# lightkurve/lightkurve

Hardware: NVIDIA H100
Metric: lombscargle_freqbins_x_cadences_per_s (higher is better)
Workload: dtype f32 spreading + FFT, f64 phase (nufft)

## Files before the change

lightkurve_b200/csrc/ls_nufft.cu:

```cuda
#include <algorithm>

#include "common.cuh"
#include "ls_common.cuh"
#include "nufft_core.h"
#include "nufft_v2.cuh"

namespace lkb {

using nufft::Cad;

namespace {

constexpr int GL_NQ = 48;
struct GlNodes {
  double x[GL_NQ], w[GL_NQ];
};

__global__ void nufft_cad_kernel(const double* __restrict__ t, int64_t N, double df, int64_t M, int w,
                                 Cad* __restrict__ cad, int* __restrict__ unsorted) {
  const int64_t n = (int64_t)blockIdx.x * blockDim.x + threadIdx.x;
  if (n >= N) return;
  cad[n] = nufft::cad_entry(t[n], df, M, w);
  if (n > 0 && t[n] < t[n - 1]) *unsorted = 1;
  if (t[n] < 0.0) *unsorted = 1;
// ... 722 lines not shown
  return LKB_OK;
}

int ls_nufft_run(const double* d_t, int64_t N, const float* d_yc, int64_t ystride, const float* d_ysumf,
                 const float* d_absmax, int B, const double* d_freq, int64_t F, const float4* d_rot,
                 const float2* d_rot2, int64_t F_low, int normalization, double norm_scale, float* d_pow,
                 cudaStream_t st, int ws_alt, bool prof) {
  const NufftPlan pl = g_plan;
  const int w = pl.w, p = pl.p;
  const float beta = pl.beta;
  const int64_t k0 = pl.k0, M = pl.M;
  const int npairs = (B + 1) / 2;
  const int mode = (pl.Wt != nullptr) ? 3 : fft_mode(p) == 3 ? 0 : fft_mode(p);
  const char* ve = getenv("LKB_NUFFT_VERIFY");
  const bool verify = ve && atoi(ve) != 0 && F_low < F;
  if (mode == 3) {
    const int64_t Mh = M >> 1;
    const size_t cells = (size_t)pl.n1max << V2_PB;
    float2 *T = nullptr, *G = nullptr;
    LKB_TRY(ws_get_t<float2>(ws_alt ? WS_OUT4 : WS_H, (size_t)B * Mh, &T));
    LKB_TRY(ws_get_t<float2>(ws_alt ? WS_OUT5 : WS_I, std::max((size_t)B * cells, verify ? (size_t)4 * Mh : (size_t)0), &G));
    unsigned* d_worst = nullptr;
    if (verify) LKB_TRY(ws_get_t<unsigned>(ws_alt ? WS_OUT7 : WS_OUT6, 1, &d_worst));
    const int ptc = V2_LOG_TILE - (p - 1 - V2_PB);
    if (prof) prof_begin(st);
    constexpr int LCS = 8;
    LKB_LAUNCH(dim3(blocks_for((int64_t)cells, 256), (unsigned)((B + LCS - 1) / LCS)), 256, st, nufft2_spread_kernel<LCS>)(
        pl.fge, pl.cad, pl.Wt, d_yc, ystride, B, w, p, ptc, pl.n1max, G);
    LKB_LAUNCH_CHECK();
    LKB_TRY(v2_cols(G, T, p, pl.n1max, B, pl.tb, st));
    const float esc_ratio = escalate_ratio();
    unsigned* d_peak = nullptr;
    int* d_list = nullptr;
    if (esc_ratio > 0.0f && F_low < F) {
      LKB_TRY(ws_get_t<unsigned>(ws_alt ? WS_Y3 : WS_Y2, (size_t)2 * B + 1, &d_peak));
      d_list = reinterpret_cast<int*>(d_peak + B);
      LKB_CUDA_CHECK(cudaMemsetAsync(d_peak, 0, sizeof(unsigned) * ((size_t)B + 1), st));
    }
    V2Finish fa;
    fa.ftab = pl.ftab; fa.k0 = k0; fa.F = F; fa.k_lo = F_low; fa.ysum = d_ysumf; fa.Nf = (float)N;
    fa.normalization = normalization; fa.scale = (float)norm_scale; fa.power = d_pow;
    fa.peak = d_peak; fa.lcmap = nullptr; fa.log2M = p;
    if (F_low < F) LKB_TRY(v2_rows(T, p, B, pl.tb, &fa, (float2*)nullptr, 0, st));
    if (F_low > 0) {
      double* acc = nullptr;
      LKB_TRY(ws_get_t<double>(ws_alt ? WS_X4 : WS_X3, (size_t)B * F_low * 2, &acc));
      LKB_CUDA_CHECK(cudaMemsetAsync(acc, 0, sizeof(double) * (size_t)B * F_low * 2, st));
// ... 3 lines not shown
          pl.lowD, N, pl.Npad, d_yc, ystride, B, (int)F_low, slice, acc);
      LKB_LAUNCH_CHECK();
      LKB_LAUNCH(blocks_for((int64_t)B * F_low, 256), 256, st, nufft2_lowfinish_kernel)(
          acc, B, (int)F_low, F, N, d_rot, d_rot2, d_ysumf, normalization, (float)norm_scale, d_pow, d_peak);
      LKB_LAUNCH_CHECK();
    }
    if (d_peak) {
      LKB_LAUNCH(blocks_for(B, 256), 256, st, nufft2_flag_kernel)(d_peak, d_absmax, B, (float)N, esc_ratio, d_list, d_list + 1,
                                                                pl.esc_total);
      LKB_LAUNCH_CHECK();
      int cap_max = 1024;
      if (const char* e = getenv("LKB_NUFFT_ESCALATE_CAP")) cap_max = std::max(1, atoi(e));
      const int cap = std::min(B, cap_max), gy = std::min(cap, 32);
      const size_t lowlen = F_low > 0 ? (size_t)F_low * 4 + (size_t)cap * F_low * 2 + cap : 0;
      double *Gbuf = nullptr;
      double2* Td = nullptr;
      LKB_TRY(ws_get_t<double>(ws_alt ? WS_Y6 : WS_Y4, 2 * (size_t)cap * cells + lowlen, &Gbuf));
      LKB_TRY(ws_get_t<double2>(ws_alt ? WS_Y7 : WS_Y5, (size_t)cap * Mh, &Td));
      double2* Gd = reinterpret_cast<double2*>(Gbuf);
      double* accW = Gbuf + 2 * (size_t)cap * cells;
      double* accY = accW + (size_t)F_low * 4;
      double* accS = accY + (size_t)cap * F_low * 2;
      const int* lst = d_list + 1;
      const int ptc_d = v2_log_tile(p - 1 - V2_PB, true) - (p - 1 - V2_PB);
      for (int base = 0; base < B; base += cap) {
        const V2Count nc = {d_list, base, cap};
        LKB_LAUNCH(dim3(blocks_for((int64_t)cells, 256), (unsigned)((gy + LCS_D - 1) / LCS_D)), 256, st,
                   nufft2_spread_list_kernel)(pl.fge, pl.cad, pl.Wtd, d_yc, ystride, lst, w, p, ptc_d, pl.n1max, Gd, nc);
        LKB_LAUNCH_CHECK();
        LKB_TRY(v2_cols(Gd, Td, p, pl.n1max, gy, pl.tbd, st, nc));
        V2Finish fd = fa;
        fd.peak = nullptr;
        fd.lcmap = lst;
        LKB_TRY(v2_rows(Td, p, gy, pl.tbd, &fd, (double2*)nullptr, 0, st, nc));
        if (F_low > 0) {
          LKB_CUDA_CHECK(cudaMemsetAsync(accW, 0, sizeof(double) * lowlen, st));
          LKB_LAUNCH(dim3((unsigned)F_low, blocks_for(N, 256 * LOWX_PER)), 256, st, nufft2_lowacc_kernel)(
              lst, nc, d_t, N, d_yc, ystride, d_freq, (int)F_low, accW, accY, accS);
          LKB_LAUNCH_CHECK();
          LKB_LAUNCH(blocks_for((int64_t)cap * F_low, 256), 256, st, nufft2_lowexact_finish_kernel)(
              lst, nc, accW, accY, accS, (int)F_low, F, N, normalization, (float)norm_scale, d_pow);
          LKB_LAUNCH_CHECK();
        }
      }
    }
    if (prof) prof_end(st);
    if (verify) {
      const int nv = std::min(B, 4);
      const int nk2 = (int)((k0 + F) >> (p - 1 - V2_PB)) + 1;
      LKB_TRY(v2_rows(T, p, nv, pl.tb, (const V2Finish*)nullptr, G, nk2, st));
      const char* fe = getenv("LKB_NUFFT_INJECT_FAULT");
// ... 145 lines not shown
  const int64_t pair = gid >> log2M, m = gid & (M - 1);
  const int64_t b0 = 2 * pair, b1 = b0 + 1;
  float2 v = make_float2(0.f, 0.f);
  {
    const int64_t po = poff[b0], n = off[b0 + 1] - off[b0];
    v.x = nufft::spread_cell_search(m, cad + po, n, y ? y + po : nullptr, y ? nufft::pow2_scale(absmax[b0]) : 1.0f, w,
                                    beta, M);
  }
  if (b1 < B) {
    const int64_t po = poff[b1], n = off[b1 + 1] - off[b1];
    v.y = nufft::spread_cell_search(m, cad + po, n, y ? y + po : nullptr, y ? nufft::pow2_scale(absmax[b1]) : 1.0f, w,
                                    beta, M);
  }
  Z[gid] = v;
}

__global__ void __launch_bounds__(256)
nufft2_spread_ragged_kernel(const Cad* __restrict__ cad, const float* __restrict__ y, const int64_t* __restrict__ off,
                            const int64_t* __restrict__ poff, int w, float beta, int p, int ptc, int n1max,
                            float2* __restrict__ G, const double* __restrict__ t, double df) {
  const int64_t cells = (int64_t)n1max << V2_PB;
  const int64_t e = (int64_t)blockIdx.x * blockDim.x + threadIdx.x;
  if (e >= cells) return;
  const int64_t M = (int64_t)1 << p, m = 2 * v2_zcell_of(e, ptc, n1max);
  const int64_t lc = blockIdx.y, po = poff[lc], n = off[lc + 1] - off[lc];
  float2 v;
  if (t) {
    const double dfM = df * (double)M;
    v.x = nufft::spread_cell_search_acc(m, cad + po, t + po, n, y ? y + po : nullptr, w, (double)beta, dfM, M);
    v.y = nufft::spread_cell_search_acc(m + 1, cad + po, t + po, n, y ? y + po : nullptr, w, (double)beta, dfM, M);
  } else {
    v.x = nufft::spread_cell_search(m, cad + po, n, y ? y + po : nullptr, 1.0f, w, beta, M);
    v.y = nufft::spread_cell_search(m + 1, cad + po, n, y ? y + po : nullptr, 1.0f, w, beta, M);
  }
  G[lc * cells + e] = v;
}

__device__ __forceinline__ float2 v2_unpack_real(const float2* __restrict__ Zn, int64_t kk, int64_t M) {
  const int64_t Mh = M >> 1;
  const float2 g1 = Zn[kk], g2 = Zn[(Mh - kk) & (Mh - 1)];
  const float2 E = make_float2(0.5f * (g1.x + g2.x), 0.5f * (g1.y - g2.y));
  const float2 O = make_float2(0.5f * (g1.y + g2.y), 0.5f * (g2.x - g1.x));
  double wsn, wcs;
  sincospi(2.0 * (double)kk / (double)M, &wsn, &wcs);
  const float wc = (float)wcs, ws = (float)wsn;
  return make_float2(E.x + wc * O.x - ws * O.y, E.y + wc * O.y + ws * O.x);
}

__device__ __forceinline__ float ragged_power(float2 hs, float2 win1, float2 win2, double Nd, double ysum,
                                              int normalization, double scale) {
  LsSums<double> d;
  d.zero();
  d.ch = (double)hs.x;
  d.sh = (double)hs.y;
  d.c = (double)win1.x;
  d.s = (double)win1.y;
  d.cc = 0.5 * (Nd + (double)win2.x);
  d.sc = 0.5 * (double)win2.y;
// ... 192 lines not shown
  const int64_t kmax = (int64_t)std::max(nterms, 1) * (k0 + F);
  const int64_t dec_first = nterms ? 0 : k0, dec_len = nterms ? kmax : F;
  LKB_TRY(ws_get_t<float2>(WS_IN4, dec_len, &dec));
  LKB_TRY(ws_get_t<float2>(WS_IN5, 2 * kmax, &dec2));
  LKB_TRY(ws_get_t<int>(WS_IN6, 1, &flag));

  LKB_CUDA_CHECK(cudaMemsetAsync(flag, 0, sizeof(int), st));
  {
    const unsigned gx = (unsigned)std::min<int64_t>(64, (nmax + 255) / 256);
    LKB_LAUNCH(dim3(gx ? gx : 1, (unsigned)B), 256, st, nufft_cad_ragged_kernel)(d_t, d_off, d_po, d_span, df, M, M2, w, cad,
                                                                          cad2, flag);
    LKB_LAUNCH_CHECK();
  }
  int h_flag = 0;
  LKB_CUDA_CHECK(cudaMemcpyAsync(&h_flag, flag, sizeof(int), cudaMemcpyDeviceToHost, st));
  LKB_CUDA_CHECK(cudaStreamSynchronize(st));
  if (h_flag) { set_error("NUFFT (ragged): a light curve has unsorted times"); return LKB_E_UNSUPPORTED; }
  LKB_LAUNCH(blocks_for(dec_len, 128), 128, st, nufft_deconv_kernel)(dec_first, dec_len, M, w, (double)beta, gl, dec);
  LKB_LAUNCH_CHECK();
  LKB_LAUNCH(blocks_for(2 * kmax, 128), 128, st, nufft_deconv_kernel)(0, 2 * kmax, M2, w, (double)beta, gl, dec2);
  LKB_LAUNCH_CHECK();

  const double* t_acc = getenv("LKB_NUFFT_RAGGED_W32") ? nullptr : d_t;
  const int ptc = V2_LOG_TILE - (p - 1 - V2_PB), ptc2 = V2_LOG_TILE - (p2 - 1 - V2_PB);
  const int nk2 = (int)(kmax >> (p - 1 - V2_PB)) + 1, nk2w = (int)((2 * kmax) >> (p2 - 1 - V2_PB)) + 1;
  prof_begin(st);
  for (int b0 = 0; b0 < B; b0 += group) {
    LKB_CHI2_OBSERVE(CHI2_PATH_GROUP);
    const int Bg = std::min(group, B - b0);
    const int64_t *off_g = d_off + b0, *po_g = d_po + b0;
    double span_min = 1e300;
    for (int b = b0; b < b0 + Bg; ++b) span_min = fmin(span_min, h_span[b]);
    const double nlow = floor((LS_LOWF_CYCLES / span_min - f0) / df) + 2.0;
    const int64_t F_low_max = nlow < 0.0 ? 0 : (nlow > (double)F ? F : (int64_t)nlow);
    LKB_LAUNCH(dim3(blocks_for((int64_t)cells2, 256), (unsigned)Bg), 256, st, nufft2_spread_ragged_kernel)(
        cad2, nullptr, off_g, po_g, w, beta, p2, ptc2, n1max2, G, t_acc, df);
    LKB_LAUNCH_CHECK();
    LKB_TRY(v2_cols(G, Tw, p2, n1max2, Bg, tb2, st));
    LKB_TRY(v2_rows(Tw, p2, Bg, tb2, nullptr, Zwn, nk2w, st));
    LKB_LAUNCH(dim3(blocks_for((int64_t)cells, 256), (unsigned)Bg), 256, st, nufft2_spread_ragged_kernel)(
        cad, d_y, off_g, po_g, w, beta, p, ptc, n1max, G, t_acc, df);
    LKB_LAUNCH_CHECK();
    LKB_TRY(v2_cols(G, T, p, n1max, Bg, tb, st));
    LKB_TRY(v2_rows(T, p, Bg, tb, nullptr, Zn, nk2, st));
    const double* ns_g = d_ns ? d_ns + b0 : nullptr;
    float* pow_g = d_pow + (size_t)b0 * F;
#define LKB_CHI2_FINISH(NT)                                                                                            \
// ... 202 lines not shown
```

lightkurve_b200/csrc/nufft_v2.cuh:

```cuda
#pragma once
#include "nufft_core.h"

namespace lkb {
namespace {

using nufft::V2_PB;
using nufft::V2_THREADS;
using nufft::V2_TILE;
constexpr int V2_LOG_TILE = 13;
static_assert((1 << V2_LOG_TILE) == V2_TILE, "tile size");
constexpr int V2_BC = 1 << V2_PB;
constexpr int V2_R = V2_TILE / (2 * V2_BC);
constexpr int V2_LSB = V2_BC + V2_BC / 16 + 1;
constexpr int V2R_P_MIN = V2_PB + 4 + 1, V2R_P_MAX = V2_PB + 13 + 1;

__host__ __device__ constexpr int v2_radix(int plog, int idx) {
  return (idx < plog / 4) ? 16 : ((idx == plog / 4 && (plog % 4)) ? (1 << (plog % 4)) : 0);
}
__host__ __device__ constexpr int v2_log2i(int r) { return r == 16 ? 4 : r == 8 ? 3 : r == 4 ? 2 : r == 2 ? 1 : 0; }
__host__ __device__ constexpr int v2_log_tile(int pa, bool dbl) { return (dbl && pa <= 12) ? 12 : V2_LOG_TILE; }
__device__ __forceinline__ int v2_skew(int a) { return a + (a >> 4); }
template <int nb>
__host__ __device__ constexpr int v2_in_off(int r) {
  return (nb % 16 == 0) ? r * (nb + nb / 16) : r * nb + ((r * nb) >> 4);
}

template <class CT>
__global__ void nufft2_tables_kernel(int pa, int pb, int ph, CT* __restrict__ tw_a, CT* __restrict__ tw_b,
                                     CT* __restrict__ t_hi, CT* __restrict__ t_lo) {
  const int la = nufft::v2_pass_table_len(pa), lb = nufft::v2_pass_table_len(pb), pl = nufft::v2_log2_lo(ph);
  const int nlo = 1 << pl, nhi = 1 << (ph - pl);
  int e = (int)(blockIdx.x * blockDim.x + threadIdx.x);
  int64_t num = 0, den = 1;
  CT* dst = nullptr;
  if (e < la) { nufft::v2_pass_table_entry(pa, e, &num, &den); dst = tw_a + e; }
  else if ((e -= la) < lb) { nufft::v2_pass_table_entry(pb, e, &num, &den); dst = tw_b + e; }
  else if ((e -= lb) < nhi) { num = e; den = nhi; dst = t_hi + e; }
  else if ((e -= nhi) < nlo) { num = e; den = (int64_t)1 << ph; dst = t_lo + e; }
  else return;
  double sn, cs;
  sincospi(2.0 * (double)num / (double)den, &sn, &cs);
  typedef typename nufft::CplxOf<CT>::real RT;
  *dst = nufft::CplxOf<CT>::mk((RT)cs, (RT)sn);
}

template <class RT>
__global__ void nufft2_weights_kernel(const double* __restrict__ t, int64_t N, double df, int64_t M, int w, double beta,
                                      RT* __restrict__ Wt) {
  const int64_t e = (int64_t)blockIdx.x * blockDim.x + threadIdx.x;
  if (e >= N * w) return;
  const int64_t n = e / w;
  const int q = (int)(e - n * w);
  const double x = df * t[n] * (double)M + (double)nufft::grid_shift(w);
  const double i0 = ceil(x - 0.5 * (double)w);
  const double z = (i0 + (double)q - x) * (2.0 / (double)w);
  const double s2 = 1.0 - z * z;
  Wt[e] = (s2 > 0.0) ? (RT)exp(beta * (sqrt(s2) - 1.0)) : (RT)0.0;
}

__device__ __forceinline__ int64_t v2_zcell_of(int64_t e, int ptc, int n1max) {
  const int64_t j = e & (((int64_t)1 << ptc) - 1), rest = e >> ptc;
  const int64_t n1 = rest % n1max, c = rest / n1max;
  return (n1 << V2_PB) + (c << ptc) + j;
}

template <int LCS>
__global__ void __launch_bounds__(256)
nufft2_spread_kernel(const int32_t* __restrict__ first_ge, const nufft::Cad* __restrict__ cad,
                     const float* __restrict__ Wt, const float* __restrict__ y, int64_t ystride, int B, int w, int p,
                     int ptc, int n1max, float2* __restrict__ G) {
  const int64_t cells = (int64_t)n1max << V2_PB;
  const int64_t e = (int64_t)blockIdx.x * blockDim.x + threadIdx.x;
  if (e >= cells) return;
  const int64_t M = (int64_t)1 << p, m = 2 * v2_zcell_of(e, ptc, n1max);
  const int lc0 = (int)blockIdx.y * LCS;
  const float* yr[LCS];
#pragma unroll
  for (int q = 0; q < LCS; ++q) {
    int b = lc0 + q;
    if (b > B - 1) b = B - 1;
    yr[q] = y + (int64_t)b * ystride;
  }
  float a0[LCS], a1[LCS];
#pragma unroll
  for (int q = 0; q < LCS; ++q) { a0[q] = 0.0f; a1[q] = 0.0f; }
  const int64_t L = nufft::table_len(M, w);
  for (int wrap = 0; wrap < 2; ++wrap) {
    const int64_t mm = m + (int64_t)wrap * M;
    if (mm + 1 >= L) break;
    int64_t lo_c = mm - w + 1, hi_c = mm + 2;
    if (lo_c < 0) lo_c = 0;
    if (hi_c > L - 1) hi_c = L - 1;
    const int32_t na = first_ge[lo_c], nb = first_ge[hi_c];
    for (int32_t n = na; n < nb; ++n) {
      const int tap = (int)(mm - (int64_t)cad[n].i0);
      const float* wr = Wt + (int64_t)n * w;
      const float w0 = (tap >= 0) ? wr[tap] : 0.0f;
      const float w1 = (tap + 1 < w) ? wr[tap + 1] : 0.0f;
#pragma unroll
      for (int q = 0; q < LCS; ++q) {
        const float v = yr[q][n];
        a0[q] = fmaf(w0, v, a0[q]);
        a1[q] = fmaf(w1, v, a1[q]);
      }
    }
  }
#pragma unroll
  for (int q = 0; q < LCS; ++q)
    if (lc0 + q < B) G[(int64_t)(lc0 + q) * cells + e] = make_float2(a0[q], a1[q]);
}

template <int PLOG, int LS, int IDX, int NS, class CT = float2, int NT = V2_THREADS>
__device__ __forceinline__ void v2_pass_t(CT* buf, const CT* __restrict__ tw, int nz = 1 << 30) {
  constexpr int R = v2_radix(PLOG, IDX);
  if constexpr (R != 0) {
    constexpr int LR = v2_log2i(R), NB = 16 / R, PNB = PLOG - LR, nb = 1 << PNB;
    constexpr bool WIDE = nb > NT;
    static_assert(WIDE || (NT % nb) == 0, "geometry");
    const int t = (int)threadIdx.x;
    CT u[NB][R];
    int base_in[NB];
#pragma unroll
    for (int q = 0; q < NB; ++q) {
      int line, i;
      if constexpr (WIDE) { line = 0; i = t + NT * q; }
      else { line = (t >> PNB) + ((NT * q) >> PNB); i = t & (nb - 1); }
      base_in[q] = line * LS + ((nb % 16 == 0) ? v2_skew(i) : i);
#pragma unroll
      for (int r = 0; r < R; ++r)
        u[q][r] = (IDX > 0 || r * nb < nz) ? buf[base_in[q] + v2_in_off<nb>(r)] : nufft::CplxOf<CT>::mk(0, 0);
    }
    __syncthreads();
#pragma unroll
    for (int q = 0; q < NB; ++q) {
      int line, i;
      if constexpr (WIDE) { line = 0; i = t + NT * q; }
      else { line = (t >> PNB) + ((NT * q) >> PNB); i = t & (nb - 1); }
      const int k = i & (NS - 1);
      if constexpr (NS > 1) {
#pragma unroll
        for (int r = 1; r < R; ++r) u[q][r] = nufft::cmul(u[q][r], tw[r * NS + k]);
      }
      nufft::SmallDft<R, CT>::run(u[q]);
      const int j = ((i - k) << LR) + k;
      const int base_out = line * LS + ((NS == 1) ? (j + i) : v2_skew(j));
#pragma unroll
      for (int r = 0; r < R; ++r) buf[base_out + ((NS == 1) ? r : r * (NS + NS / 16))] = u[q][r];
    }
    __syncthreads();
    v2_pass_t<PLOG, LS, IDX + 1, NS * R, CT, NT>(buf, tw + ((IDX > 0) ? R * NS : 0));
  }
}

struct V2Count {
  const int* count;
  int base, cap;
};
__device__ __forceinline__ int v2_count(const V2Count nc, int grid_y) {
  if (!nc.count) return grid_y;
  const int n = *nc.count - nc.base;
  return n < 0 ? 0 : (n > nc.cap ? nc.cap : n);
}

template <int PA, class CT, int LOGT = V2_LOG_TILE>
__device__ __forceinline__ void v2_cols_one(CT* buf, const CT* __restrict__ G, CT* __restrict__ T, int n1max,
                                            const CT* __restrict__ tw_a, const CT* __restrict__ t_hi,
                                            const CT* __restrict__ t_lo, const int64_t lc) {
  constexpr int NT = (1 << LOGT) / 16;
  constexpr int A = 1 << PA, PTC = LOGT - PA, TC = 1 << PTC, LS = A + A / 16 + 1, C = V2_BC / TC;
  constexpr int JW = TC < NT / 16 ? TC : NT / 16, RW = NT / JW, CG = TC / JW;
  constexpr int LJW = JW == 32 ? 5 : JW == 16 ? 4 : JW == 8 ? 3 : JW == 4 ? 2 : JW == 2 ? 1 : 0;
  static_assert((1 << LJW) == JW && RW % 16 == 0, "geometry");
  const int t = (int)threadIdx.x, c = (int)blockIdx.x;
  const int jl = t & (JW - 1), nl = t >> LJW;
  const int nvalid = n1max << PTC;
  const CT* Gp = G + (lc * C + c) * (int64_t)nvalid;
  const int s_base = jl * LS + v2_skew(nl), g_base = nl * TC + jl;
  constexpr int NB1 = A / v2_radix(PA, 0);
  const int nz = ((n1max + NB1 - 1) / NB1) * NB1;
#pragma unroll
  for (int u = 0; u < 16; ++u) {
    const int cg = u % CG, nbk = u / CG;
    if (nbk * RW < nz) {
      const int idx = g_base + nbk * RW * TC + cg * JW;
      buf[s_base + cg * JW * LS + nbk * (RW + RW / 16)] = (idx < nvalid) ? Gp[idx] : nufft::CplxOf<CT>::mk(0, 0);
    }
  }
  __syncthreads();
  v2_pass_t<PA, LS, 0, 1, CT, NT>(buf, tw_a, nz);
  CT* Tp = T + (lc * C + c) * (int64_t)(1 << LOGT);
  const int ph = PA + V2_PB, pl = nufft::v2_log2_lo(ph);
  const unsigned Mmask = (1u << ph) - 1u, lmask = (1u << pl) - 1u;
#pragma unroll
  for (int u = 0; u < 16; ++u) {
    const int cg = u % CG, nbk = u / CG;
    const int k1 = nl + nbk * RW, n2 = c * TC + jl + cg * JW;
    const unsigned q = ((unsigned)n2 * (unsigned)k1) & Mmask;
    const CT wq = nufft::cmul(t_hi[q >> pl], t_lo[q & lmask]);
    Tp[g_base + nbk * RW * TC + cg * JW] = nufft::cmul(buf[s_base + cg * JW * LS + nbk * (RW + RW / 16)], wq);
  }
}
template <int PA, class CT = float2>
__global__ void __launch_bounds__(V2_THREADS, sizeof(CT) == 8 ? 2 : 1)
nufft2_cols_kernel(const CT* __restrict__ G, CT* __restrict__ T, int n1max, const CT* __restrict__ tw_a,
                   const CT* __restrict__ t_hi, const CT* __restrict__ t_lo) {
  LKB_DYN_SMEM(CT, buf);
  v2_cols_one<PA, CT>(buf, G, T, n1max, tw_a, t_hi, t_lo, (int64_t)blockIdx.y);
}
template <int PA, int LOGT>
__device__ __noinline__ void v2_cols_list_one(double2* buf, const double2* __restrict__ G, double2* __restrict__ T,
                                              int n1max, const double2* __restrict__ tw_a,
                                              const double2* __restrict__ t_hi, const double2* __restrict__ t_lo,
                                              const int64_t lc) {
  v2_cols_one<PA, double2, LOGT>(buf, G, T, n1max, tw_a, t_hi, t_lo, lc);
}
template <int PA, int LOGT = v2_log_tile(PA, true)>
__global__ void __launch_bounds__((1 << LOGT) / 16, LOGT < V2_LOG_TILE ? 2 : 1)
nufft2_cols_list_kernel(const double2* __restrict__ G, double2* __restrict__ T, int n1max,
                        const double2* __restrict__ tw_a, const double2* __restrict__ t_hi,
                        const double2* __restrict__ t_lo, V2Count nc) {
  LKB_DYN_SMEM(double2, buf);
  const int64_t ntr = v2_count(nc, (int)gridDim.y);
  for (int64_t lc = blockIdx.y; lc < ntr; lc += gridDim.y) {
    __syncthreads();
    v2_cols_list_one<PA, LOGT>(buf, G, T, n1max, tw_a, t_hi, t_lo, lc);
  }
}

struct V2FTab {
  float4 d;
  float4 c;
};
struct V2Finish {
  const V2FTab* ftab;
  int64_t k0, F, k_lo;
  const float* ysum;
  float Nf;
  int normalization;
  float scale;
// ... 6 lines not shown
__device__ __forceinline__ float v2_normalise(float pw, float Nf, int normalization, float scale) {
  if (normalization == LKB_LS_NORM_PSD_SCALE) return pw * scale;
  if (normalization == LKB_LS_NORM_AMPLITUDE) return sqrtf(pw * (4.0f / Nf));
  return pw;
}
__device__ __forceinline__ float v2_finish_pw(float2 g1, float2 g2, const V2FTab tb, float ysum, int64_t, int) {
  const float ex = 0.5f * (g1.x + g2.x), ey = 0.5f * (g1.y - g2.y);
  const float ox = 0.5f * (g1.y + g2.y), oy = 0.5f * (g2.x - g1.x);
  const float yc = ex * tb.d.x - ey * tb.d.y + ox * tb.d.z - oy * tb.d.w - ysum * tb.c.x;
  const float ys = ex * tb.d.y + ey * tb.d.x + ox * tb.d.w + oy * tb.d.z - ysum * tb.c.y;
  return yc * yc * tb.c.z + ys * ys * tb.c.w;
}
__device__ __forceinline__ float v2_finish_pw(double2 g1, double2 g2, const V2FTab tb, float ysum, int64_t kk, int log2M) {
  const double ex = 0.5 * (g1.x + g2.x), ey = 0.5 * (g1.y - g2.y);
  const double ox = 0.5 * (g1.y + g2.y), oy = 0.5 * (g2.x - g1.x);
  double sw, cw;
  sincospi(ldexp((double)kk, 1 - log2M), &sw, &cw);
  const double gx = ex + cw * ox - sw * oy, gy = ey + cw * oy + sw * ox;
  const double yc = gx * (double)tb.d.x - gy * (double)tb.d.y - (double)ysum * (double)tb.c.x;
  const double ys = gx * (double)tb.d.y + gy * (double)tb.d.x - (double)ysum * (double)tb.c.y;
  return (float)(yc * yc * (double)tb.c.z + ys * ys * (double)tb.c.w);
}

template <int PA, int MODE, class CT, int LOGT = V2_LOG_TILE>
__device__ __forceinline__ void v2_rows_one(CT* buf, const CT* __restrict__ T, const CT* __restrict__ tw_b,
                                            const V2Finish& fa, CT* __restrict__ Zout, int nk2_keep, const int64_t lc,
                                            const int lc_base, const int g) {
  constexpr int NT = (1 << LOGT) / 16, R = (1 << LOGT) / (2 * V2_BC), LR = v2_log2i(R);
  constexpr int A = 1 << PA, PTC = LOGT - PA, TC = 1 << PTC, LS = V2_LSB, Bc = V2_BC;
  static_assert((1 << LR) == R, "geometry");
  const int t = (int)threadIdx.x;
  const bool last = g == (A / (2 * R)) - 1;
  const int64_t Mh = (int64_t)1 << (PA + V2_PB);
  auto slot_k1 = [&](int s) -> int {
    const int h = s >> LR, r = s & (R - 1);
    if (h == 0) return 1 + g * R + r;
    if (last && r == 0) return 0;
    return A - (g + 1) * R + r;
  };
  const CT* Tp = T + lc * Mh;
#pragma unroll
  for (int u = 0; u < 16; ++u) {
    const int e = t + NT * u;
    const int j = e & (TC - 1), r = (e >> PTC) & (R - 1), h = (e >> (PTC + LR)) & 1, c = e >> (PTC + LR + 1);
    const int s = h * R + r;
    buf[s * LS + v2_skew((c << PTC) + j)] = Tp[(((c << PA) + slot_k1(s)) << PTC) + j];
  }
  __syncthreads();
  v2_pass_t<V2_PB, LS, 0, 1, CT, NT>(buf, tw_b);
  constexpr int KSTEP = NT / (2 * R);
  const int s = t & (2 * R - 1), h = s >> LR, r = s & (R - 1), k1 = slot_k1(s);
  if (MODE == 2) {
    const int keep = nk2_keep < Bc / 2 ? nk2_keep : Bc / 2;
    for (int q = t >> (LR + 1); q < 2 * keep; q += KSTEP) {
      const int k2 = q < keep ? q : Bc - 2 * keep + q;
      Zout[lc * Mh + k1 + ((int64_t)k2 << PA)] = buf[s * LS + v2_skew(k2)];
    }
  } else {
  int ps = (1 - h) * R + (R - 1 - r);
  bool row0 = false;
  if (last && h == 0 && r == R - 1) ps = s;
  if (last && h == 1 && r == 0) { ps = s; row0 = true; }
  int64_t nK2 = ((fa.k0 + fa.F - 1) >> PA) + 1;
  if (nK2 > Bc) nK2 = Bc;
  const int64_t lcd = fa.lcmap ? (int64_t)fa.lcmap[lc_base + lc] : lc;
  const float ys0 = fa.ysum[lcd];
  float* prow = fa.power + lcd * fa.F;
  const int64_t jbase = (int64_t)k1 - fa.k0;
  float pmax = 0.0f;
  constexpr int UB = 4;
  for (int k2b = t >> (LR + 1); k2b < (int)nK2; k2b += KSTEP * UB) {
    V2FTab tb[UB];
// ... 5 lines not shown
      jj[u] = jbase + ((int64_t)k2 << PA);
      valid[u] = k2 < (int)nK2 && jj[u] >= fa.k_lo && jj[u] < fa.F;
      if (valid[u]) tb[u] = fa.ftab[jj[u]];
    }
#pragma unroll
    for (int u = 0; u < UB; ++u) {
      if (!valid[u]) continue;
      const int k2 = k2b + KSTEP * u;
      const int pi = row0 ? ((Bc - k2) & (Bc - 1)) : (Bc - 1 - k2);
      const CT g1 = buf[s * LS + v2_skew(k2)], g2 = buf[ps * LS + v2_skew(pi)];
      const float pw = v2_finish_pw(g1, g2, tb[u], ys0, fa.k0 + jj[u], fa.log2M);
      pmax = fmaxf(pmax, pw);
      prow[jj[u]] = v2_normalise(pw, fa.Nf, fa.normalization, fa.scale);
    }
  }
  if (fa.peak) {
#pragma unroll
    for (int o = 16; o > 0; o >>= 1) pmax = fmaxf(pmax, __shfl_xor_sync(0xffffffffu, pmax, o));
    if ((t & 31) == 0 && pmax > 0.0f) atomicMax(fa.peak + lcd, __float_as_uint(pmax));
  }
  }
}

template <int PA, int MODE, class CT = float2>
__global__ void __launch_bounds__(V2_THREADS, sizeof(CT) == 8 ? 2 : 1)
nufft2_rows_kernel(const CT* __restrict__ T, const CT* __restrict__ tw_b, V2Finish fa, CT* __restrict__ Zout,
                   int nk2_keep) {
  LKB_DYN_SMEM(CT, buf);
  v2_rows_one<PA, MODE, CT>(buf, T, tw_b, fa, Zout, nk2_keep, (int64_t)blockIdx.y, 0, (int)blockIdx.x);
}
template <int PA, int LOGT>
__device__ __noinline__ void v2_rows_list_one(double2* buf, const double2* __restrict__ T,
                                              const double2* __restrict__ tw_b, const V2Finish fa, const int64_t lc,
                                              const int lc_base) {
  v2_rows_one<PA, 1, double2, LOGT>(buf, T, tw_b, fa, nullptr, 0, lc, lc_base, (int)blockIdx.x);
}
template <int PA, int LOGT = v2_log_tile(PA, true)>
__global__ void __launch_bounds__((1 << LOGT) / 16, LOGT < V2_LOG_TILE ? 2 : 1)
nufft2_rows_list_kernel(const double2* __restrict__ T, const double2* __restrict__ tw_b, V2Finish fa, V2Count nc) {
  LKB_DYN_SMEM(double2, buf);
  const int64_t ntr = v2_count(nc, (int)gridDim.y);
  for (int64_t lc = blockIdx.y; lc < ntr; lc += gridDim.y) {
    __syncthreads();
    v2_rows_list_one<PA, LOGT>(buf, T, tw_b, fa, lc, nc.base);
  }
}

__global__ void nufft2_flag_kernel(const unsigned* __restrict__ peak, const float* __restrict__ absmax, int B, float Nf,
                                   float ratio, int* __restrict__ count, int* __restrict__ list, int* __restrict__ total) {
  const int b = (int)(blockIdx.x * blockDim.x + threadIdx.x);
  bool f = false;
  if (b < B) {
    const float amp = sqrtf(__uint_as_float(peak[b]) * (4.0f / Nf));
    f = absmax[b] > ratio * amp;
  }
  const unsigned bal = __ballot_sync(0xffffffffu, f);
  if (bal) {
    int base = 0;
    if ((threadIdx.x & 31) == 0) {
      base = atomicAdd(count, __popc(bal));
// ... 62 lines not shown
template <class CT>
inline int v2_tables(int p, int slot, cudaStream_t st, V2TablesT<CT>* out) {
  const int ph = p - 1, pa = ph - V2_PB, pl = nufft::v2_log2_lo(ph);
  const int la = nufft::v2_pass_table_len(pa), lb = nufft::v2_pass_table_len(V2_PB), nhi = 1 << (ph - pl), nlo = 1 << pl;
  CT* base = nullptr;
  LKB_TRY(ws_get_t<CT>(slot, (size_t)(la + lb + nhi + nlo + 4), &base));
  CT *tw_a = base, *tw_b = base + la, *t_hi = tw_b + lb, *t_lo = t_hi + nhi;
  LKB_LAUNCH(v2_blocks_for(la + lb + nhi + nlo, 256), 256, st, nufft2_tables_kernel<CT>)(pa, V2_PB, ph, tw_a, tw_b, t_hi, t_lo);
  LKB_LAUNCH_CHECK();
  out->tw_a = tw_a; out->tw_b = tw_b; out->t_hi = t_hi; out->t_lo = t_lo;
  return LKB_OK;
}
inline int v2_n1max(int p, int64_t i0_last, int w) {
  const int64_t M = (int64_t)1 << p, A = (M / 2) >> V2_PB;
  const int64_t reach = i0_last + w + 1;
  if (reach >= M) return (int)A;
  const int64_t n = ((reach + 1) / 2 + V2_BC - 1) >> V2_PB;
  return (int)(n < 1 ? 1 : (n > A ? A : n));
}
inline bool v2_supported(int p) { return p >= V2R_P_MIN && p <= V2R_P_MAX; }

template <int PA, class CT>
int v2_cols_pa(const CT* G, CT* T, int n1max, int B, const V2TablesT<CT>& tb, cudaStream_t st, V2Count nc) {
  constexpr int LOGT = v2_log_tile(PA, sizeof(CT) == 16), A = 1 << PA, TC = (1 << LOGT) / A;
  const size_t smem = (size_t)TC * (A + A / 16 + 1) * sizeof(CT);
  const dim3 grid((unsigned)(V2_BC / TC), (unsigned)B);
  if constexpr (sizeof(CT) == 16) {
    LKB_CUDA_CHECK(cudaFuncSetAttribute(nufft2_cols_list_kernel<PA>, cudaFuncAttributeMaxDynamicSharedMemorySize, (int)smem));
    LKB_LAUNCH_SMEM(grid, (1 << LOGT) / 16, smem, st, nufft2_cols_list_kernel<PA>)(G, T, n1max, tb.tw_a, tb.t_hi, tb.t_lo, nc);
  } else {
    LKB_CUDA_CHECK(cudaFuncSetAttribute(nufft2_cols_kernel<PA, CT>, cudaFuncAttributeMaxDynamicSharedMemorySize, (int)smem));
    LKB_LAUNCH_SMEM(grid, V2_THREADS, smem, st, nufft2_cols_kernel<PA, CT>)(G, T, n1max, tb.tw_a, tb.t_hi, tb.t_lo);
  }
  LKB_LAUNCH_CHECK();
  return LKB_OK;
}
template <int PA, class CT>
int v2_rows_pa(const CT* T, int B, const V2TablesT<CT>& tb, const V2Finish* fa, CT* Zout, int nk2_keep, cudaStream_t st,
               V2Count nc) {
  constexpr int LOGT = v2_log_tile(PA, sizeof(CT) == 16), R = (1 << LOGT) / (2 * V2_BC);
  const size_t smem = (size_t)(2 * R) * V2_LSB * sizeof(CT);
  const dim3 grid((unsigned)((1 << PA) / (2 * R)), (unsigned)B);
  if constexpr (sizeof(CT) == 16) {
    LKB_CUDA_CHECK(cudaFuncSetAttribute(nufft2_rows_list_kernel<PA>, cudaFuncAttributeMaxDynamicSharedMemorySize, (int)smem));
    LKB_LAUNCH_SMEM(grid, (1 << LOGT) / 16, smem, st, nufft2_rows_list_kernel<PA>)(T, tb.tw_b, *fa, nc);
  } else {
    LKB_CUDA_CHECK(cudaFuncSetAttribute(nufft2_rows_kernel<PA, 1, CT>, cudaFuncAttributeMaxDynamicSharedMemorySize, (int)smem));
    LKB_CUDA_CHECK(cudaFuncSetAttribute(nufft2_rows_kernel<PA, 2, CT>, cudaFuncAttributeMaxDynamicSharedMemorySize, (int)smem));
    if (fa) LKB_LAUNCH_SMEM(grid, V2_THREADS, smem, st, nufft2_rows_kernel<PA, 1, CT>)(T, tb.tw_b, *fa, nullptr, 0);
    else LKB_LAUNCH_SMEM(grid, V2_THREADS, smem, st, nufft2_rows_kernel<PA, 2, CT>)(T, tb.tw_b, V2Finish(), Zout, nk2_keep);
  }
  LKB_LAUNCH_CHECK();
  return LKB_OK;
}
#define V2_DISPATCH_PA(pa, CALL)                                                                       \
  switch (pa) {                                                                                         \
    case 4: return CALL(4); case 5: return CALL(5); case 6: return CALL(6); case 7: return CALL(7);      \
    case 8: return CALL(8); case 9: return CALL(9); case 10: return CALL(10); case 11: return CALL(11);  \
    case 12: return CALL(12); case 13: return CALL(13);                                                  \
    default: set_error("NUFFT v2: fine grid of 2^%d cells out of range", (pa) + V2_PB + 1); return LKB_E_UNSUPPORTED; \
  }
template <class CT>
inline int v2_cols(const CT* G, CT* T, int p, int n1max, int B, const V2TablesT<CT>& tb, cudaStream_t st,
                   V2Count nc = V2Count{nullptr, 0, 0}) {
#define V2_CALL(PA) v2_cols_pa<PA, CT>(G, T, n1max, B, tb, st, nc)
  V2_DISPATCH_PA(p - 1 - V2_PB, V2_CALL)
#undef V2_CALL
}
template <class CT>
inline int v2_rows(const CT* T, int p, int B, const V2TablesT<CT>& tb, const V2Finish* fa, CT* Zout, int nk2_keep,
                   cudaStream_t st, V2Count nc = V2Count{nullptr, 0, 0}) {
#define V2_CALL(PA) v2_rows_pa<PA, CT>(T, B, tb, fa, Zout, nk2_keep, st, nc)
  V2_DISPATCH_PA(p - 1 - V2_PB, V2_CALL)
// ... 6 lines not shown
```

lightkurve_b200/csrc/ptx.cuh:

```cuda
#pragma once
#include <stdint.h>
#include <cuda.h>

namespace lkb {
namespace ptx {

__device__ __forceinline__ uint32_t smem_u32(const void* p) {
  return static_cast<uint32_t>(__cvta_generic_to_shared(p));
}

__device__ __forceinline__ void mbar_init(uint64_t* bar, uint32_t count) {
  asm volatile("mbarrier.init.shared::cta.b64 [%0], %1;" ::"r"(smem_u32(bar)), "r"(count) : "memory");
}
__device__ __forceinline__ void mbar_fence_init() {
  asm volatile("fence.mbarrier_init.release.cluster;" ::: "memory");
}
__device__ __forceinline__ void mbar_arrive_expect_tx(uint64_t* bar, uint32_t bytes) {
  asm volatile("mbarrier.arrive.expect_tx.shared::cta.b64 _, [%0], %1;" ::"r"(smem_u32(bar)), "r"(bytes)
               : "memory");
}
__device__ __forceinline__ void mbar_arrive(uint64_t* bar) {
  asm volatile("mbarrier.arrive.shared::cta.b64 _, [%0];" ::"r"(smem_u32(bar)) : "memory");
}
__device__ __forceinline__ bool mbar_try_wait(uint64_t* bar, uint32_t parity) {
// ... 22 lines not shown
  while (!mbar_try_wait_hint(bar, parity, hint_ns)) {
  }
}
__device__ __forceinline__ void mbar_wait(uint64_t* bar, uint32_t parity) {
  while (!mbar_try_wait(bar, parity)) {
  }
}
__device__ __forceinline__ void mbar_wait_sleep(uint64_t* bar, uint32_t parity, uint32_t ns) {
  while (!mbar_try_wait(bar, parity)) {
    if (ns) __nanosleep(ns);
  }
}

__device__ __forceinline__ void fence_proxy_async_smem() {
  asm volatile("fence.proxy.async.shared::cta;" ::: "memory");
}
__device__ __forceinline__ void bulk_g2s(void* dst_smem, const void* src_gmem, uint32_t bytes, uint64_t* bar) {
  asm volatile(
      "cp.async.bulk.shared::cluster.global.mbarrier::complete_tx::bytes [%0], [%1], %2, [%3];" ::"r"(
          smem_u32(dst_smem)),
      "l"(src_gmem), "r"(bytes), "r"(smem_u32(bar))
      : "memory");
}
__device__ __forceinline__ void tma_load_2d(void* dst_smem, const CUtensorMap* map, int32_t c0, int32_t c1,
                                            uint64_t* bar) {
  asm volatile(
      "cp.async.bulk.tensor.2d.shared::cluster.global.tile.mbarrier::complete_tx::bytes [%0], [%1, {%3, %4}], [%2];" ::
          "r"(smem_u32(dst_smem)),
      "l"(map), "r"(smem_u32(bar)), "r"(c0), "r"(c1)
      : "memory");
}
__device__ __forceinline__ void prefetch_tensormap(const CUtensorMap* map) {
  asm volatile("prefetch.tensormap [%0];" ::"l"(map) : "memory");
}

template <int N>
__device__ __forceinline__ void setmaxnreg_dec() { asm volatile("setmaxnreg.dec.sync.aligned.u32 %0;" ::"n"(N)); }
template <int N>
__device__ __forceinline__ void setmaxnreg_inc() { asm volatile("setmaxnreg.inc.sync.aligned.u32 %0;" ::"n"(N)); }

__device__ __forceinline__ uint64_t wgmma_desc_k64b(uint32_t smem_addr) {
  uint64_t d = 0;
  d |= (uint64_t)((smem_addr >> 4) & 0x3FFF);
  d |= (uint64_t)1 << 16;
  d |= (uint64_t)(512 >> 4) << 32;
  d |= (uint64_t)2 << 62;
// ... 29 lines not shown
```

Before: 1664000 billion.

## Use bulk async copies and column-major G layout in NUFFT FFT passes

```diff
diff --git a/lightkurve_b200/csrc/ls_nufft.cu b/lightkurve_b200/csrc/ls_nufft.cu
--- a/lightkurve_b200/csrc/ls_nufft.cu
+++ b/lightkurve_b200/csrc/ls_nufft.cu
@@ -768,7 +768,7 @@
     LKB_TRY(ws_get_t<float2>(ws_alt ? WS_OUT5 : WS_I, std::max((size_t)B * cells, verify ? (size_t)4 * Mh : (size_t)0), &G));
     unsigned* d_worst = nullptr;
     if (verify) LKB_TRY(ws_get_t<unsigned>(ws_alt ? WS_OUT7 : WS_OUT6, 1, &d_worst));
-    const int ptc = V2_LOG_TILE - (p - 1 - V2_PB);
+    const int ptc = v2_log_tile(p - 1 - V2_PB) - (p - 1 - V2_PB);
     if (prof) prof_begin(st);
     constexpr int LCS = 8;
     LKB_LAUNCH(dim3(blocks_for((int64_t)cells, 256), (unsigned)((B + LCS - 1) / LCS)), 256, st, nufft2_spread_kernel<LCS>)(
@@ -818,11 +818,10 @@
       double* accY = accW + (size_t)F_low * 4;
       double* accS = accY + (size_t)cap * F_low * 2;
       const int* lst = d_list + 1;
-      const int ptc_d = v2_log_tile(p - 1 - V2_PB, true) - (p - 1 - V2_PB);
       for (int base = 0; base < B; base += cap) {
         const V2Count nc = {d_list, base, cap};
         LKB_LAUNCH(dim3(blocks_for((int64_t)cells, 256), (unsigned)((gy + LCS_D - 1) / LCS_D)), 256, st,
-                   nufft2_spread_list_kernel)(pl.fge, pl.cad, pl.Wtd, d_yc, ystride, lst, w, p, ptc_d, pl.n1max, Gd, nc);
+                   nufft2_spread_list_kernel)(pl.fge, pl.cad, pl.Wtd, d_yc, ystride, lst, w, p, ptc, pl.n1max, Gd, nc);
         LKB_LAUNCH_CHECK();
         LKB_TRY(v2_cols(Gd, Td, p, pl.n1max, gy, pl.tbd, st, nc));
         V2Finish fd = fa;
@@ -1014,7 +1013,7 @@
   const int64_t cells = (int64_t)n1max << V2_PB;
   const int64_t e = (int64_t)blockIdx.x * blockDim.x + threadIdx.x;
   if (e >= cells) return;
-  const int64_t M = (int64_t)1 << p, m = 2 * v2_zcell_of(e, ptc, n1max);
+  const int64_t M = (int64_t)1 << p, m = 2 * e;
   const int64_t lc = blockIdx.y, po = poff[lc], n = off[lc + 1] - off[lc];
   float2 v;
   if (t) {
@@ -1025,7 +1024,7 @@
     v.x = nufft::spread_cell_search(m, cad + po, n, y ? y + po : nullptr, 1.0f, w, beta, M);
     v.y = nufft::spread_cell_search(m + 1, cad + po, n, y ? y + po : nullptr, 1.0f, w, beta, M);
   }
-  G[lc * cells + e] = v;
+  G[lc * cells + v2_gpos_of(e, ptc, n1max)] = v;
 }
 
 __device__ __forceinline__ float2 v2_unpack_real(const float2* __restrict__ Zn, int64_t kk, int64_t M) {
@@ -1264,7 +1263,7 @@
   LKB_LAUNCH_CHECK();
 
   const double* t_acc = getenv("LKB_NUFFT_RAGGED_W32") ? nullptr : d_t;
-  const int ptc = V2_LOG_TILE - (p - 1 - V2_PB), ptc2 = V2_LOG_TILE - (p2 - 1 - V2_PB);
+  const int ptc = v2_log_tile(p - 1 - V2_PB) - (p - 1 - V2_PB), ptc2 = v2_log_tile(p2 - 1 - V2_PB) - (p2 - 1 - V2_PB);
   const int nk2 = (int)(kmax >> (p - 1 - V2_PB)) + 1, nk2w = (int)((2 * kmax) >> (p2 - 1 - V2_PB)) + 1;
   prof_begin(st);
   for (int b0 = 0; b0 < B; b0 += group) {
diff --git a/lightkurve_b200/csrc/nufft_v2.cuh b/lightkurve_b200/csrc/nufft_v2.cuh
--- a/lightkurve_b200/csrc/nufft_v2.cuh
+++ b/lightkurve_b200/csrc/nufft_v2.cuh
@@ -1,5 +1,10 @@
 #pragma once
 #include "nufft_core.h"
+#ifndef LKB_CUDA_EMU
+#include "ptx.cuh"
+#else
+#include "ptx_emu.h"
+#endif
 
 namespace lkb {
 namespace {
@@ -10,7 +15,6 @@
 constexpr int V2_LOG_TILE = 13;
 static_assert((1 << V2_LOG_TILE) == V2_TILE, "tile size");
 constexpr int V2_BC = 1 << V2_PB;
-constexpr int V2_R = V2_TILE / (2 * V2_BC);
 constexpr int V2_LSB = V2_BC + V2_BC / 16 + 1;
 constexpr int V2R_P_MIN = V2_PB + 4 + 1, V2R_P_MAX = V2_PB + 13 + 1;
 
@@ -18,7 +22,8 @@
   return (idx < plog / 4) ? 16 : ((idx == plog / 4 && (plog % 4)) ? (1 << (plog % 4)) : 0);
 }
 __host__ __device__ constexpr int v2_log2i(int r) { return r == 16 ? 4 : r == 8 ? 3 : r == 4 ? 2 : r == 2 ? 1 : 0; }
-__host__ __device__ constexpr int v2_log_tile(int pa, bool dbl) { return (dbl && pa <= 12) ? 12 : V2_LOG_TILE; }
+__host__ __device__ constexpr int v2_log_tile(int pa) { return pa <= 12 ? 12 : V2_LOG_TILE; }
+__host__ __device__ constexpr int v2_ctas_per_sm(int logt) { return 1024 >> (logt - 4); }
 __device__ __forceinline__ int v2_skew(int a) { return a + (a >> 4); }
 template <int nb>
 __host__ __device__ constexpr int v2_in_off(int r) {
@@ -63,6 +68,10 @@
   const int64_t n1 = rest % n1max, c = rest / n1max;
   return (n1 << V2_PB) + (c << ptc) + j;
 }
+__device__ __forceinline__ int64_t v2_gpos_of(int64_t n, int ptc, int n1max) {
+  const int64_t n1 = n >> V2_PB, n2 = n & (V2_BC - 1);
+  return ((((n2 >> ptc) * n1max) + n1) << ptc) + (n2 & (((int64_t)1 << ptc) - 1));
+}
 
 template <int LCS>
 __global__ void __launch_bounds__(256)
@@ -72,7 +81,7 @@
   const int64_t cells = (int64_t)n1max << V2_PB;
   const int64_t e = (int64_t)blockIdx.x * blockDim.x + threadIdx.x;
   if (e >= cells) return;
-  const int64_t M = (int64_t)1 << p, m = 2 * v2_zcell_of(e, ptc, n1max);
+  const int64_t M = (int64_t)1 << p, m = 2 * e, ge = v2_gpos_of(e, ptc, n1max);
   const int lc0 = (int)blockIdx.y * LCS;
   const float* yr[LCS];
 #pragma unroll
@@ -107,11 +116,14 @@
   }
 #pragma unroll
   for (int q = 0; q < LCS; ++q)
-    if (lc0 + q < B) G[(int64_t)(lc0 + q) * cells + e] = make_float2(a0[q], a1[q]);
-}
-
-template <int PLOG, int LS, int IDX, int NS, class CT = float2, int NT = V2_THREADS>
-__device__ __forceinline__ void v2_pass_t(CT* buf, const CT* __restrict__ tw, int nz = 1 << 30) {
+    if (lc0 + q < B) G[(int64_t)(lc0 + q) * cells + ge] = make_float2(a0[q], a1[q]);
+}
+
+struct V2SkewIn {
+  static constexpr bool dense = false;
+};
+template <int PLOG, int LS, int IDX, int NS, class CT = float2, int NT = V2_THREADS, class IN = V2SkewIn>
+__device__ __forceinline__ void v2_pass_t(CT* buf, const CT* __restrict__ tw, int nz = 1 << 30, IN in = IN()) {
   constexpr int R = v2_radix(PLOG, IDX);
   if constexpr (R != 0) {
     constexpr int LR = v2_log2i(R), NB = 16 / R, PNB = PLOG - LR, nb = 1 << PNB;
@@ -127,8 +139,10 @@
       else { line = (t >> PNB) + ((NT * q) >> PNB); i = t & (nb - 1); }
       base_in[q] = line * LS + ((nb % 16 == 0) ? v2_skew(i) : i);
 #pragma unroll
-      for (int r = 0; r < R; ++r)
-        u[q][r] = (IDX > 0 || r * nb < nz) ? buf[base_in[q] + v2_in_off<nb>(r)] : nufft::CplxOf<CT>::mk(0, 0);
+      for (int r = 0; r < R; ++r) {
+        if constexpr (IDX == 0 && IN::dense) u[q][r] = buf[in(line, i + r * nb)];
+        else u[q][r] = (IDX > 0 || r * nb < nz) ? buf[base_in[q] + v2_in_off<nb>(r)] : nufft::CplxOf<CT>::mk(0, 0);
+      }
     }
     __syncthreads();
 #pragma unroll
@@ -162,7 +176,7 @@
   return n < 0 ? 0 : (n > nc.cap ? nc.cap : n);
 }
 
-template <int PA, class CT, int LOGT = V2_LOG_TILE>
+template <int PA, class CT, int LOGT>
 __device__ __forceinline__ void v2_cols_one(CT* buf, const CT* __restrict__ G, CT* __restrict__ T, int n1max,
                                             const CT* __restrict__ tw_a, const CT* __restrict__ t_hi,
                                             const CT* __restrict__ t_lo, const int64_t lc) {
@@ -191,21 +205,39 @@
   CT* Tp = T + (lc * C + c) * (int64_t)(1 << LOGT);
   const int ph = PA + V2_PB, pl = nufft::v2_log2_lo(ph);
   const unsigned Mmask = (1u << ph) - 1u, lmask = (1u << pl) - 1u;
-#pragma unroll
-  for (int u = 0; u < 16; ++u) {
+  auto twiddled = [&](int u) -> CT {
     const int cg = u % CG, nbk = u / CG;
     const int k1 = nl + nbk * RW, n2 = c * TC + jl + cg * JW;
     const unsigned q = ((unsigned)n2 * (unsigned)k1) & Mmask;
     const CT wq = nufft::cmul(t_hi[q >> pl], t_lo[q & lmask]);
-    Tp[g_base + nbk * RW * TC + cg * JW] = nufft::cmul(buf[s_base + cg * JW * LS + nbk * (RW + RW / 16)], wq);
-  }
-}
-template <int PA, class CT = float2>
-__global__ void __launch_bounds__(V2_THREADS, sizeof(CT) == 8 ? 2 : 1)
+    return nufft::cmul(buf[s_base + cg * JW * LS + nbk * (RW + RW / 16)], wq);
+  };
+  auto t_pos = [&](int u) { return g_base + (u / CG) * RW * TC + (u % CG) * JW; };
+  if constexpr (sizeof(CT) == 8) {
+    CT v[16];
+#pragma unroll
+    for (int u = 0; u < 16; ++u) v[u] = twiddled(u);
+    __syncthreads();
+#pragma unroll
+    for (int u = 0; u < 16; ++u) buf[t_pos(u)] = v[u];
+    ptx::fence_proxy_async_smem();
+    __syncthreads();
+    if (t == 0) {
+      ptx::bulk_s2g(Tp, buf, (uint32_t)((1 << LOGT) * sizeof(CT)));
+      ptx::bulk_commit();
+      ptx::bulk_wait_read();
+    }
+  } else {
+#pragma unroll
+    for (int u = 0; u < 16; ++u) Tp[t_pos(u)] = twiddled(u);
+  }
+}
+template <int PA, class CT = float2, int LOGT = v2_log_tile(PA)>
+__global__ void __launch_bounds__((1 << LOGT) / 16, v2_ctas_per_sm(LOGT))
 nufft2_cols_kernel(const CT* __restrict__ G, CT* __restrict__ T, int n1max, const CT* __restrict__ tw_a,
                    const CT* __restrict__ t_hi, const CT* __restrict__ t_lo) {
   LKB_DYN_SMEM(CT, buf);
-  v2_cols_one<PA, CT>(buf, G, T, n1max, tw_a, t_hi, t_lo, (int64_t)blockIdx.y);
+  v2_cols_one<PA, CT, LOGT>(buf, G, T, n1max, tw_a, t_hi, t_lo, (int64_t)blockIdx.y);
 }
 template <int PA, int LOGT>
 __device__ __noinline__ void v2_cols_list_one(double2* buf, const double2* __restrict__ G, double2* __restrict__ T,
@@ -214,7 +246,7 @@
                                               const int64_t lc) {
   v2_cols_one<PA, double2, LOGT>(buf, G, T, n1max, tw_a, t_hi, t_lo, lc);
 }
-template <int PA, int LOGT = v2_log_tile(PA, true)>
+template <int PA, int LOGT = v2_log_tile(PA)>
 __global__ void __launch_bounds__((1 << LOGT) / 16, LOGT < V2_LOG_TILE ? 2 : 1)
 nufft2_cols_list_kernel(const double2* __restrict__ G, double2* __restrict__ T, int n1max,
                         const double2* __restrict__ tw_a, const double2* __restrict__ t_hi,
@@ -267,12 +299,25 @@
   return (float)(yc * yc * (double)tb.c.z + ys * ys * (double)tb.c.w);
 }
 
-template <int PA, int MODE, class CT, int LOGT = V2_LOG_TILE>
+template <int PTC, int LR>
+struct V2RowsDenseIn {
+  static constexpr bool dense = true;
+  __device__ __forceinline__ int operator()(int s, int n2) const {
+    return ((((n2 >> PTC) << (LR + 1)) + s) << PTC) + (n2 & ((1 << PTC) - 1));
+  }
+};
+template <class CT, int PTC>
+constexpr bool v2_rows_bulk() { return sizeof(CT) == 8 && PTC >= 1; }
+template <class CT, int LOGT>
+constexpr size_t v2_rows_smem() {
+  return (size_t)((1 << LOGT) / V2_BC) * V2_LSB * sizeof(CT) + (sizeof(CT) == 8 ? sizeof(uint64_t) : 0);
+}
+template <int PA, int MODE, class CT, int LOGT>
 __device__ __forceinline__ void v2_rows_one(CT* buf, const CT* __restrict__ T, const CT* __restrict__ tw_b,
                                             const V2Finish& fa, CT* __restrict__ Zout, int nk2_keep, const int64_t lc,
                                             const int lc_base, const int g) {
   constexpr int NT = (1 << LOGT) / 16, R = (1 << LOGT) / (2 * V2_BC), LR = v2_log2i(R);
-  constexpr int A = 1 << PA, PTC = LOGT - PA, TC = 1 << PTC, LS = V2_LSB, Bc = V2_BC;
+  constexpr int A = 1 << PA, PTC = v2_log_tile(PA) - PA, TC = 1 << PTC, LS = V2_LSB, Bc = V2_BC;
   static_assert((1 << LR) == R, "geometry");
   const int t = (int)threadIdx.x;
   const bool last = g == (A / (2 * R)) - 1;
@@ -284,15 +329,40 @@
     return A - (g + 1) * R + r;
   };
   const CT* Tp = T + lc * Mh;
-#pragma unroll
-  for (int u = 0; u < 16; ++u) {
-    const int e = t + NT * u;
-    const int j = e & (TC - 1), r = (e >> PTC) & (R - 1), h = (e >> (PTC + LR)) & 1, c = e >> (PTC + LR + 1);
-    const int s = h * R + r;
-    buf[s * LS + v2_skew((c << PTC) + j)] = Tp[(((c << PA) + slot_k1(s)) << PTC) + j];
-  }
-  __syncthreads();
-  v2_pass_t<V2_PB, LS, 0, 1, CT, NT>(buf, tw_b);
+  if constexpr (v2_rows_bulk<CT, PTC>()) {
+    constexpr int C = Bc / TC;
+    constexpr uint32_t ROWB = TC * sizeof(CT);
+    uint64_t* bar = reinterpret_cast<uint64_t*>(buf + 2 * R * LS);
+    if (t == 0) {
+      ptx::mbar_init(bar, 1);
+      ptx::mbar_fence_init();
+      ptx::mbar_arrive_expect_tx(bar, 2 * R * Bc * (uint32_t)sizeof(CT));
+    }
+    __syncthreads();
+    for (int q = t; q < 2 * C; q += NT) {
+      const int c = q >> 1, h = q & 1;
+      CT* dst = buf + q * R * TC;
+      const CT* src = Tp + (((c << PA) + slot_k1(h * R)) << PTC);
+      if (h == 1 && last) {
+        ptx::bulk_g2s(dst, src, ROWB, bar);
+        ptx::bulk_g2s(dst + TC, Tp + (((c << PA) + slot_k1(R + 1)) << PTC), (R - 1) * ROWB, bar);
+      } else {
+        ptx::bulk_g2s(dst, src, R * ROWB, bar);
+      }
+    }
+    ptx::mbar_wait(bar, 0);
+    v2_pass_t<V2_PB, LS, 0, 1, CT, NT>(buf, tw_b, 1 << 30, V2RowsDenseIn<PTC, LR>());
+  } else {
+#pragma unroll
+    for (int u = 0; u < 16; ++u) {
+      const int e = t + NT * u;
+      const int j = e & (TC - 1), r = (e >> PTC) & (R - 1), h = (e >> (PTC + LR)) & 1, c = e >> (PTC + LR + 1);
+      const int s = h * R + r;
+      buf[s * LS + v2_skew((c << PTC) + j)] = Tp[(((c << PA) + slot_k1(s)) << PTC) + j];
+    }
+    __syncthreads();
+    v2_pass_t<V2_PB, LS, 0, 1, CT, NT>(buf, tw_b);
+  }
   constexpr int KSTEP = NT / (2 * R);
   const int s = t & (2 * R - 1), h = s >> LR, r = s & (R - 1), k1 = slot_k1(s);
   if (MODE == 2) {
@@ -344,12 +414,12 @@
   }
 }
 
-template <int PA, int MODE, class CT = float2>
-__global__ void __launch_bounds__(V2_THREADS, sizeof(CT) == 8 ? 2 : 1)
+template <int PA, int MODE, class CT = float2, int LOGT = V2_LOG_TILE>
+__global__ void __launch_bounds__((1 << LOGT) / 16, v2_ctas_per_sm(LOGT))
 nufft2_rows_kernel(const CT* __restrict__ T, const CT* __restrict__ tw_b, V2Finish fa, CT* __restrict__ Zout,
                    int nk2_keep) {
   LKB_DYN_SMEM(CT, buf);
-  v2_rows_one<PA, MODE, CT>(buf, T, tw_b, fa, Zout, nk2_keep, (int64_t)blockIdx.y, 0, (int)blockIdx.x);
+  v2_rows_one<PA, MODE, CT, LOGT>(buf, T, tw_b, fa, Zout, nk2_keep, (int64_t)blockIdx.y, 0, (int)blockIdx.x);
 }
 template <int PA, int LOGT>
 __device__ __noinline__ void v2_rows_list_one(double2* buf, const double2* __restrict__ T,
@@ -357,7 +427,7 @@
                                               const int lc_base) {
   v2_rows_one<PA, 1, double2, LOGT>(buf, T, tw_b, fa, nullptr, 0, lc, lc_base, (int)blockIdx.x);
 }
-template <int PA, int LOGT = v2_log_tile(PA, true)>
+template <int PA, int LOGT = v2_log_tile(PA)>
 __global__ void __launch_bounds__((1 << LOGT) / 16, LOGT < V2_LOG_TILE ? 2 : 1)
 nufft2_rows_list_kernel(const double2* __restrict__ T, const double2* __restrict__ tw_b, V2Finish fa, V2Count nc) {
   LKB_DYN_SMEM(double2, buf);
@@ -466,7 +536,7 @@
 
 template <int PA, class CT>
 int v2_cols_pa(const CT* G, CT* T, int n1max, int B, const V2TablesT<CT>& tb, cudaStream_t st, V2Count nc) {
-  constexpr int LOGT = v2_log_tile(PA, sizeof(CT) == 16), A = 1 << PA, TC = (1 << LOGT) / A;
+  constexpr int LOGT = v2_log_tile(PA), A = 1 << PA, TC = (1 << LOGT) / A;
   const size_t smem = (size_t)TC * (A + A / 16 + 1) * sizeof(CT);
   const dim3 grid((unsigned)(V2_BC / TC), (unsigned)B);
   if constexpr (sizeof(CT) == 16) {
@@ -474,7 +544,7 @@
     LKB_LAUNCH_SMEM(grid, (1 << LOGT) / 16, smem, st, nufft2_cols_list_kernel<PA>)(G, T, n1max, tb.tw_a, tb.t_hi, tb.t_lo, nc);
   } else {
     LKB_CUDA_CHECK(cudaFuncSetAttribute(nufft2_cols_kernel<PA, CT>, cudaFuncAttributeMaxDynamicSharedMemorySize, (int)smem));
-    LKB_LAUNCH_SMEM(grid, V2_THREADS, smem, st, nufft2_cols_kernel<PA, CT>)(G, T, n1max, tb.tw_a, tb.t_hi, tb.t_lo);
+    LKB_LAUNCH_SMEM(grid, (1 << LOGT) / 16, smem, st, nufft2_cols_kernel<PA, CT>)(G, T, n1max, tb.tw_a, tb.t_hi, tb.t_lo);
   }
   LKB_LAUNCH_CHECK();
   return LKB_OK;
@@ -482,8 +552,8 @@
 template <int PA, class CT>
 int v2_rows_pa(const CT* T, int B, const V2TablesT<CT>& tb, const V2Finish* fa, CT* Zout, int nk2_keep, cudaStream_t st,
                V2Count nc) {
-  constexpr int LOGT = v2_log_tile(PA, sizeof(CT) == 16), R = (1 << LOGT) / (2 * V2_BC);
-  const size_t smem = (size_t)(2 * R) * V2_LSB * sizeof(CT);
+  constexpr int LOGT = sizeof(CT) == 16 ? v2_log_tile(PA) : V2_LOG_TILE, R = (1 << LOGT) / (2 * V2_BC);
+  const size_t smem = v2_rows_smem<CT, LOGT>();
   const dim3 grid((unsigned)((1 << PA) / (2 * R)), (unsigned)B);
   if constexpr (sizeof(CT) == 16) {
     LKB_CUDA_CHECK(cudaFuncSetAttribute(nufft2_rows_list_kernel<PA>, cudaFuncAttributeMaxDynamicSharedMemorySize, (int)smem));
@@ -491,8 +561,8 @@
   } else {
     LKB_CUDA_CHECK(cudaFuncSetAttribute(nufft2_rows_kernel<PA, 1, CT>, cudaFuncAttributeMaxDynamicSharedMemorySize, (int)smem));
     LKB_CUDA_CHECK(cudaFuncSetAttribute(nufft2_rows_kernel<PA, 2, CT>, cudaFuncAttributeMaxDynamicSharedMemorySize, (int)smem));
-    if (fa) LKB_LAUNCH_SMEM(grid, V2_THREADS, smem, st, nufft2_rows_kernel<PA, 1, CT>)(T, tb.tw_b, *fa, nullptr, 0);
-    else LKB_LAUNCH_SMEM(grid, V2_THREADS, smem, st, nufft2_rows_kernel<PA, 2, CT>)(T, tb.tw_b, V2Finish(), Zout, nk2_keep);
+    if (fa) LKB_LAUNCH_SMEM(grid, (1 << LOGT) / 16, smem, st, nufft2_rows_kernel<PA, 1, CT>)(T, tb.tw_b, *fa, nullptr, 0);
+    else LKB_LAUNCH_SMEM(grid, (1 << LOGT) / 16, smem, st, nufft2_rows_kernel<PA, 2, CT>)(T, tb.tw_b, V2Finish(), Zout, nk2_keep);
   }
   LKB_LAUNCH_CHECK();
   return LKB_OK;
diff --git a/lightkurve_b200/csrc/ptx.cuh b/lightkurve_b200/csrc/ptx.cuh
--- a/lightkurve_b200/csrc/ptx.cuh
+++ b/lightkurve_b200/csrc/ptx.cuh
@@ -68,6 +68,13 @@
       "l"(src_gmem), "r"(bytes), "r"(smem_u32(bar))
       : "memory");
 }
+__device__ __forceinline__ void bulk_s2g(void* dst_gmem, const void* src_smem, uint32_t bytes) {
+  asm volatile("cp.async.bulk.global.shared::cta.bulk_group [%0], [%1], %2;" ::"l"(dst_gmem), "r"(smem_u32(src_smem)),
+               "r"(bytes)
+               : "memory");
+}
+__device__ __forceinline__ void bulk_commit() { asm volatile("cp.async.bulk.commit_group;" ::: "memory"); }
+__device__ __forceinline__ void bulk_wait_read() { asm volatile("cp.async.bulk.wait_group.read 0;" ::: "memory"); }
 __device__ __forceinline__ void tma_load_2d(void* dst_smem, const CUtensorMap* map, int32_t c0, int32_t c1,
                                             uint64_t* bar) {
   asm volatile(
diff --git a/lightkurve_b200/csrc/ptx_emu.h b/lightkurve_b200/csrc/ptx_emu.h
--- /dev/null
+++ b/lightkurve_b200/csrc/ptx_emu.h
@@ -0,0 +1,46 @@
+#pragma once
+#include <stdint.h>
+#include <stdio.h>
+#include <stdlib.h>
+#include <string.h>
+
+#include <thread>
+
+namespace lkb {
+namespace ptx {
+
+inline int* emu_mbar(uint64_t* bar) { return reinterpret_cast<int*>(bar); }
+inline void emu_bulk_check(const void* a, const void* b, uint32_t bytes) {
+  if ((bytes % 16) || ((uintptr_t)a % 16) || ((uintptr_t)b % 16)) {
+    fprintf(stderr, "ptx_emu: bulk copy of %u bytes between %p and %p is not 16-byte aligned\n", bytes, a, b);
+    abort();
+  }
+}
+inline void mbar_init(uint64_t* bar, uint32_t count) {
+  __atomic_store_n(&emu_mbar(bar)[1], 0, __ATOMIC_SEQ_CST);
+  __atomic_store_n(&emu_mbar(bar)[0], (int)count, __ATOMIC_SEQ_CST);
+}
+inline void mbar_fence_init() {}
+inline void mbar_arrive_expect_tx(uint64_t* bar, uint32_t bytes) {
+  __atomic_add_fetch(&emu_mbar(bar)[1], (int)bytes, __ATOMIC_SEQ_CST);
+  __atomic_sub_fetch(&emu_mbar(bar)[0], 1, __ATOMIC_SEQ_CST);
+}
+inline void mbar_wait(uint64_t* bar, uint32_t) {
+  while (__atomic_load_n(&emu_mbar(bar)[0], __ATOMIC_SEQ_CST) != 0 || __atomic_load_n(&emu_mbar(bar)[1], __ATOMIC_SEQ_CST) != 0)
+    std::this_thread::yield();
+}
+inline void bulk_g2s(void* dst_smem, const void* src_gmem, uint32_t bytes, uint64_t* bar) {
+  emu_bulk_check(dst_smem, src_gmem, bytes);
+  memcpy(dst_smem, src_gmem, bytes);
+  __atomic_sub_fetch(&emu_mbar(bar)[1], (int)bytes, __ATOMIC_SEQ_CST);
+}
+inline void fence_proxy_async_smem() {}
+inline void bulk_s2g(void* dst_gmem, const void* src_smem, uint32_t bytes) {
+  emu_bulk_check(dst_gmem, src_smem, bytes);
+  memcpy(dst_gmem, src_smem, bytes);
+}
+inline void bulk_commit() {}
+inline void bulk_wait_read() {}
+
+}
+}
```

After: 1839000 billion (median of 6 runs). +10.5%, better.
